# Banus/pano360

Measured on AMD Instinct MI355X. Metric: blended megapixels/sec (multiband), higher is better.
Workload: dtype f32; 1 GPU; cfg3: 32 synthetic 3840x2160 frames per image set, spherical warp + multiband blend L=5, native resolution (MAX_RESOLUTION uncapped); frames=32

## Files before the change

### pano360_amd/csrc/blend.hip

```cpp
#include <stdlib.h>

#include "geom.h"

__global__ __launch_bounds__(256) void ownership_kernel(
    const pano_patch *__restrict__ patches, int n, int H, int W,
    int16_t *__restrict__ owner, uint8_t *__restrict__ valid) {
    const int x = blockIdx.x * 64 + threadIdx.x, y = blockIdx.y * 4 + threadIdx.y;
    if (x >= W || y >= H) return;
    float best = 0.0f;
    int who = -1;
    bool any = false;
    for (int i = 0; i < n; ++i) {
        const pano_patch p = patches[i];
        const int px = x - p.x0, py = y - p.y0;
        if ((unsigned)px >= (unsigned)p.w || (unsigned)py >= (unsigned)p.h) continue;
        const float a = p.planes[3 * (size_t)p.vh * p.vpitch + (size_t)py * p.vpitch + px];
        if (a > best) {
            best = a;
            who = i;
        }
        any |= p.mask[(size_t)py * p.w + px] == 0;
    }
    owner[(size_t)y * W + x] = (int16_t)who;
    valid[(size_t)y * W + x] = any ? 1 : 0;
}

#define OWN_LIST 256

struct CamList {
    int list[OWN_LIST];
    int wave[4];
    int count;
};

__device__ __forceinline__ int build_camera_list(CamList &sh, const pano_camera *__restrict__ cams,
                                                 int n, int bx0, int bx1, int by0, int by1) {
    const int tid = threadIdx.y * 64 + threadIdx.x, lane = threadIdx.x, wave = threadIdx.y;
    if (tid == 0) sh.count = 0;
    __syncthreads();
    bool overflow = false;
    for (int base = 0; base < n; base += 256) {
        const int i = base + tid;
        bool hit = false;
        if (i < n) {
            const pano_camera *cam = cams + i;
            hit = cam->x0 < bx1 && cam->x0 + cam->w > bx0 && cam->y0 < by1 && cam->y0 + cam->h > by0;
        }
        const unsigned long long bal = __ballot(hit);
        if (lane == 0) sh.wave[wave] = __popcll(bal);
        __syncthreads();
        int off = sh.count;
        for (int w = 0; w < wave; ++w) off += sh.wave[w];
        const int total = sh.count + sh.wave[0] + sh.wave[1] + sh.wave[2] + sh.wave[3];
        off += __popcll(bal & ((1ull << lane) - 1ull));
        if (hit && off < OWN_LIST) sh.list[off] = i;
        __syncthreads();
        if (tid == 0) sh.count = total;
        if (total > OWN_LIST) overflow = true;
        __syncthreads();
    }
    return overflow ? -1 : sh.count;
}

struct AlphaBound {
    float lo, hi;
};

__device__ __forceinline__ void hat_range(double a, double b, int n, double &lo, double &hi) {
    const double mid = 0.5 * n, peak = fmin(fmax(mid, a), b);
    hi = 0.5 - fabs(peak - mid) / n;
    lo = fmin(0.5 - fabs(a - mid) / n, 0.5 - fabs(b - mid) / n);
}

__device__ __forceinline__ void iv_axpy(double k, double lo, double hi, double &alo, double &ahi) {
    alo += k >= 0.0 ? k * lo : k * hi;
    ahi += k >= 0.0 ? k * hi : k * lo;
}

__device__ __forceinline__ AlphaBound alpha_bound_of(const pano_camera *cam, const double (*v)[2]);

__device__ __forceinline__ AlphaBound alpha_bound(const pano_camera *cam, const double *r) {
    const double *K = cam->proj;
    double v[3][2];
#pragma unroll
    for (int row = 0; row < 3; ++row) {
        double lo = 0.0, hi = 0.0;
        iv_axpy(K[3 * row + 0], r[0], r[1], lo, hi);
        iv_axpy(K[3 * row + 1], r[2], r[3], lo, hi);
        iv_axpy(K[3 * row + 2], r[4], r[5], lo, hi);
        const double slack = 1e-9 * (fabs(lo) + fabs(hi)) + 1e-300;
        v[row][0] = lo - slack;
        v[row][1] = hi + slack;
    }
    return alpha_bound_of(cam, v);
}

__device__ __forceinline__ AlphaBound alpha_bound_ends(const pano_camera *cam, double sa, double ca,
                                                       double sb, double cb, double t_lo,
                                                       double t_hi) {
    const double *K = cam->proj;
    const double chord2 = (sb - sa) * (sb - sa) + (cb - ca) * (cb - ca);
    double v[3][2];
#pragma unroll
    for (int row = 0; row < 3; ++row) {
        const double a = K[3 * row + 0], b = K[3 * row + 2];
        const double ga = a * sa + b * ca, gb = a * sb + b * cb;
        const double e = (fabs(a) + fabs(b)) * chord2 * 0.1258;
        double lo = fmin(ga, gb) - e, hi = fmax(ga, gb) + e;
        iv_axpy(K[3 * row + 1], t_lo, t_hi, lo, hi);
        const double slack = 1e-9 * (fabs(lo) + fabs(hi) + fabs(ga) + fabs(gb)) + 1e-300;
        v[row][0] = lo - slack;
        v[row][1] = hi + slack;
    }
    return alpha_bound_of(cam, v);
}

__device__ __forceinline__ AlphaBound alpha_bound_of(const pano_camera *cam, const double (*v)[2]) {
    AlphaBound out;
    if (v[2][1] <= 0.0) {
        out.lo = 0.0f;
        out.hi = -1.0f;
        return out;
    }
    if (v[2][0] <= 1e-6 * (fabs(v[0][0]) + fabs(v[0][1]) + fabs(v[1][0]) + fabs(v[1][1]) + 1.0)) {
        out.lo = 0.0f;
        out.hi = 1.0f;
        return out;
    }
    const int sw = cam->sw, sh = cam->sh;
    double box[2][2];
#pragma unroll
    for (int a = 0; a < 2; ++a) {
        const double q0 = v[a][0] / v[2][0], q1 = v[a][0] / v[2][1];
        const double q2 = v[a][1] / v[2][0], q3 = v[a][1] / v[2][1];
        const double half = 0.5 * (a == 0 ? sw : sh);
        box[a][0] = fmin(fmin(q0, q1), fmin(q2, q3)) + half - 2.0;
        box[a][1] = fmax(fmax(q0, q1), fmax(q2, q3)) + half + 2.0;
    }
    if (box[0][1] < 0.0 || box[0][0] > sw - 1.0 || box[1][1] < 0.0 || box[1][0] > sh - 1.0) {
        out.lo = 0.0f;
        out.hi = -1.0f;
        return out;
    }
    const bool inside = box[0][0] >= 0.0 && box[0][1] <= sw - 1.0 && box[1][0] >= 0.0 &&
                        box[1][1] <= sh - 1.0;
    double xlo, xhi, ylo, yhi;
    hat_range(fmax(box[0][0], 0.0), fmin(box[0][1], sw - 1.0), sw, xlo, xhi);
    hat_range(fmax(box[1][0], 0.0), fmin(box[1][1], sh - 1.0), sh, ylo, yhi);
    out.hi = (float)(fmax(xhi, 0.0) * fmax(yhi, 0.0) * (1.0 + 1e-6)) + 1e-7f;
    out.lo = inside ? fmaxf((float)(fmax(xlo, 0.0) * fmax(ylo, 0.0) * (1.0 - 1e-6)) - 1e-7f, 0.0f)
                    : 0.0f;
    return out;
}
// ... 363 lines not shown
        owned_box_pixel(o, x, y, top || row[x - W] != o, bottom || row[x + W] != o,
                        x == xs0 || row[x - 1] != o, x == xs1 - 1 || row[x + 1] != o, W, boxes,
                        stride, marks);
    }
}

__device__ __forceinline__ uint8_t quant255(float v) { return (uint8_t)(int)(255.0f * v); }

#define IB PANO_INTERIOR_BLOCK

__global__ __launch_bounds__(256) void block_owner_kernel(const int16_t *__restrict__ owner,
                                                          int H, int W, int xs0, int xs1,
                                                          int H8, int W8, int blo, int bhi,
                                                          int16_t *__restrict__ bown) {
    const int bx = blo + blockIdx.x * 64 + threadIdx.x, by = blockIdx.y * 4 + threadIdx.y;
    if (bx >= bhi || by >= H8) return;
    const int x0 = bx * IB, y0 = by * IB;
    int o = -2;
    if (x0 >= xs0 && (x0 + IB < W ? x0 + IB : W) <= xs1) {
        o = owner[(size_t)y0 * W + x0];
        const bool whole = x0 + IB <= W && (W & 1) == 0;
        if (x0 + IB <= W && y0 + IB <= H) {
            static_assert(IB == 4, "one 8-byte load per block row");
            typedef uint64_t u64_any __attribute__((aligned(2)));
            const uint64_t o16 = (uint16_t)o;
            const uint64_t all = o16 | o16 << 16 | o16 << 32 | o16 << 48;
            uint64_t diff = 0;
#pragma unroll
            for (int dy = 0; dy < IB; ++dy)
                diff |= *(const u64_any *)(owner + (size_t)(y0 + dy) * W + x0) ^ all;
            if (diff) o = -2;
        } else
        for (int dy = 0; dy < IB && o != -2; ++dy) {
            const int y = y0 + dy;
            if (y >= H) break;
            if (whole) {
                const uint32_t *q = (const uint32_t *)(owner + (size_t)y * W + x0);
                const uint32_t both = ((uint32_t)(uint16_t)o << 16) | (uint16_t)o;
                uint32_t diff = 0;
#pragma unroll
                for (int k = 0; k < IB / 2; ++k) diff |= q[k] ^ both;
                if (diff) o = -2;
            } else {
                for (int dx = 0; dx < IB; ++dx) {
                    const int x = x0 + dx;
                    if (x >= W) break;
                    if (owner[(size_t)y * W + x] != o) {
                        o = -2;
                        break;
                    }
                }
            }
        }
    }
    bown[(size_t)by * W8 + bx] = (int16_t)o;
}

#define IT_W 64
#define IT_H 16
#define IT_REACH_MAX 20
__device__ __forceinline__ bool agree(int a, int b) { return a == b || a == -3 || b == -3; }

struct LevelReaches {
    int n;
    int reach[PANO_MAX_LEVELS];
};

__global__ __launch_bounds__(256) void interior_tile_kernel(const int16_t *__restrict__ bown,
                                                            int H8, int W8, int reach, int blo,
                                                            int bhi, int ilo, int ihi,
                                                            uint8_t *__restrict__ interior,
                                                            LevelReaches lv,
                                                            uint8_t *__restrict__ classes) {
    __shared__ int16_t s_own[(IT_H + 2 * IT_REACH_MAX) * (IT_W + 2 * IT_REACH_MAX)];
    __shared__ int16_t s_col[IT_H * (IT_W + 2 * IT_REACH_MAX)];
    __shared__ unsigned long long s_vmask[IT_W + 2 * IT_REACH_MAX];
    const int tid = threadIdx.x, lane = tid & 63, wave = tid >> 6;
    const int bx0 = ilo + blockIdx.x * IT_W, by0 = blockIdx.y * IT_H;
    const int tw = IT_W + 2 * reach, th = IT_H + 2 * reach;
    for (int ty = wave; ty < th; ty += 4) {
        const int y = by0 - reach + ty;
        const bool row_in = y >= 0 && y < H8;
        for (int tx = lane; tx < tw; tx += 64) {
            const int x = bx0 - reach + tx;
            s_own[ty * tw + tx] = (row_in && x >= 0 && x < W8)
                                      ? (x >= blo && x < bhi ? bown[(size_t)y * W8 + x] : (int16_t)-2)
                                      : (int16_t)-3;
        }
    }
    __syncthreads();
    for (int tx = tid; tx < tw; tx += 256) {
        unsigned long long m = 0;
        int prev = s_own[tx];
#pragma unroll 8
        for (int ty = 0; ty + 1 < th; ++ty) {
            const int cur = s_own[(ty + 1) * tw + tx];
            m |= (unsigned long long)agree(prev, cur) << ty;
            prev = cur;
        }
        s_vmask[tx] = m;
    }
    __syncthreads();
    int cls[IT_H / 4];
#pragma unroll
    for (int r = 0; r < IT_H / 4; ++r) cls[r] = 0;
    const int nlv = classes ? lv.n : 1;
    for (int q = 0; q < nlv; ++q) {
        const int rq = classes ? lv.reach[q] : reach, off = reach - rq;
        const unsigned long long full = (1ull << (2 * rq)) - 1ull;
        for (int ry = wave; ry < IT_H; ry += 4)
            for (int tx = lane; tx < tw; tx += 64) {
                const int o = s_own[(ry + reach) * tw + tx];
                const bool same = ((s_vmask[tx] >> (ry + off)) & full) == full;
                s_col[ry * tw + tx] = (int16_t)(o >= 0 && !same ? -2 : o);
            }
        __syncthreads();
#pragma unroll
        for (int r = 0; r < IT_H / 4; ++r) {
            const int ry = wave + 4 * r;
            const int16_t *row = s_col + ry * tw;
            const int a0 = row[lane], a1 = row[min(lane + 1, tw - 1)];
            const int b0 = row[min(lane + 64, tw - 1)], b1 = row[min(lane + 65, tw - 1)];
            const unsigned long long lo = __ballot(lane + 1 < tw && agree(a0, a1));
            const unsigned long long hi = __ballot(lane + 65 < tw && agree(b0, b1));
            const int sh = lane + off;
            const unsigned long long win = sh == 0 ? lo
                                           : sh < 64 ? (lo >> sh) | (hi << (64 - sh))
                                                     : hi >> (sh - 64);
            const int o = row[lane + reach];
            if (o >= 0 && (win & full) == full && cls[r] == q) cls[r] = q + 1;
        }
        __syncthreads();
    }
#pragma unroll
    for (int r = 0; r < IT_H / 4; ++r) {
        const int y = by0 + wave + 4 * r, x = bx0 + lane;
        if (y >= H8 || x >= ihi) continue;
        interior[(size_t)y * W8 + x] = cls[r] == nlv ? 1 : 0;
        if (classes) classes[(size_t)y * W8 + x] = (uint8_t)cls[r];
    }
}

struct InteriorArgs {
    const uint8_t *interior;
    int W8;
    const pano_camera *cams;
    const double *sin_t, *cos_t, *tan_p;
    const float *lut;
    const uint8_t *classes;
};

enum { LUT_LDS = 0, LUT_GLOBAL = 1 };

template <int LUT>
__device__ __forceinline__ void shade_interior(const pano_camera *cam, const float *__restrict__ table,
                                               const InteriorArgs &ia, int x, int y, int W,
                                               uint8_t *__restrict__ mosaic,
                                               float *__restrict__ mosaic_f32) {
    if (!cam->frame) return;
    const int sw = cam->sw, sh = cam->sh;
    float fx, fy;
    map_pixel(cam->proj, table_f64(ia.sin_t, x), table_f64(ia.cos_t, x), table_f64(ia.tan_p, y), sw, sh, fx, fy);
    Taps tp = tap_base(fx, fy);
    TapBytes tb;
    if (__ballot(!taps_interior(tp, sw, sh)) == 0ull) {
        tb = load_taps_interior(cam->frame, sw, tp);
    } else {
        tp.x1 = min(tp.x1, sw - 1);
        tp.y1 = min(tp.y1, sh - 1);
        tb = load_taps(cam->frame, sw, tp);
    }
    const size_t g = ((size_t)y * W + x) * 3;
#pragma unroll
    for (int c = 0; c < 3; ++c) {
        float v = lerp4(lut_at(table, tb.v[0][c]), lut_at(table, tb.v[1][c]),
                        lut_at(table, tb.v[2][c]), lut_at(table, tb.v[3][c]), tp);
        v = v < 0.0f ? 0.0f : (v > 1.0f ? 1.0f : v);
        if (mosaic_f32) mosaic_f32[g + c] = v;
        mosaic[g + c] = (uint8_t)(int)(255.0f * v);
    }
}

template <int LUT>
__device__ __forceinline__ void shade_interior_of(int own, const float *__restrict__ table, int stride,
                                                  const InteriorArgs &ia, int x, int y, int W,
                                                  uint8_t *__restrict__ mosaic,
                                                  float *__restrict__ mosaic_f32) {
    const int own_u = __builtin_amdgcn_readfirstlane(own);
    if (__ballot(own != own_u) == 0)
        shade_interior<LUT>(ia.cams + own_u, table + (size_t)own_u * stride, ia, x, y, W, mosaic, mosaic_f32);
    else
        shade_interior<LUT>(ia.cams + own, table + (size_t)own * stride, ia, x, y, W, mosaic, mosaic_f32);
}

#define COMPOSE_MASKS 4
template <int L, bool PERCAM, bool CLS>
__global__ __launch_bounds__(256) void multiband_compose_kernel(
    const pano_patch *__restrict__ patches, int n, int H, int W, int xs0, int xs1,
    const int16_t *__restrict__ owner, const uint8_t *__restrict__ valid,
    uint8_t *__restrict__ mosaic, float *__restrict__ mosaic_f32, InteriorArgs ia) {
    __shared__ float s_lut[256];
    if (ia.interior && !PERCAM) {
        s_lut[threadIdx.y * 64 + threadIdx.x] = ia.lut[threadIdx.y * 64 + threadIdx.x];
        __syncthreads();
    }
    const int x = xs0 + blockIdx.x * 64 + threadIdx.x, y = blockIdx.y * 4 + threadIdx.y;
    const bool inside = x < xs1 && y < H;
    const bool is_interior = inside && ia.interior && ia.interior[(size_t)(y / IB) * ia.W8 + x / IB];
    unsigned long long cand[COMPOSE_MASKS] = {};
    const bool masked = n <= 64 * COMPOSE_MASKS && __ballot(inside && !is_interior) != 0;
    if (masked) {
        const int wx0 = xs0 + blockIdx.x * 64, wx1 = min(wx0 + 64, xs1);
#pragma unroll
        for (int m = 0; m < COMPOSE_MASKS; ++m) {
            const int i = 64 * m + (int)threadIdx.x;
            bool hit = false;
            if (i < n) {
                const pano_patch *q = patches + i;
                const int ax = q->x0 + q->ax0, ay = q->y0 + q->ay0;
                hit = ax < wx1 && ax + q->aw > wx0 && ay <= y && y < ay + q->ah;
            }
            cand[m] = __ballot(hit);
        }
    }
    if (!inside) return;
    if (is_interior) {
        const int own = owner[(size_t)y * W + x];
        if (PERCAM)
            shade_interior_of<LUT_GLOBAL>(own, ia.lut, 256, ia, x, y, W, mosaic, mosaic_f32);
        else
            shade_interior_of<LUT_LDS>(own, s_lut, 0, ia, x, y, W, mosaic, mosaic_f32);
        return;
    }
    float layer[L][3], wsum[L];
#pragma unroll
    for (int k = 0; k < L; ++k) layer[k][0] = layer[k][1] = layer[k][2] = wsum[k] = 0.0f;
    const int j = CLS && L > 1 ? (int)ia.classes[(size_t)(y / IB) * ia.W8 + x / IB] : 0;
    const int own_px = CLS && j > 0 ? (int)owner[(size_t)y * W + x] : -1;
    float base[3] = {0.0f, 0.0f, 0.0f};

    int m = 0;
    unsigned long long bits = masked ? cand[0] : 0ull;
    for (int i = 0;; ++i) {
        if (masked) {
            while (bits == 0ull && ++m < COMPOSE_MASKS) bits = cand[m];
            if (bits == 0ull) break;
            i = 64 * m + __ffsll((long long)bits) - 1;
            bits &= bits - 1ull;
        } else if (i >= n) {
            break;
        }
        const pano_patch p = patches[i];
        const int ax = x - p.x0 - p.ax0, ay = y - p.y0 - p.ay0;
        if ((unsigned)ax >= (unsigned)p.aw || (unsigned)ay >= (unsigned)p.ah) continue;
        const size_t vplane = (size_t)p.vh * p.vpitch;
        const size_t vo = (size_t)(ay + p.ay0 - p.vy0) * p.vpitch + (ax + p.ax0 - p.vx0);
        const size_t aplane = (size_t)p.ah * p.apitch, ao = (size_t)ay * p.apitch + ax;
        float hi[3], ha = 0.0f;
        if (!CLS || j == 0) {
#pragma unroll
            for (int c = 0; c < 3; ++c) hi[c] = p.planes[c * vplane + vo];
        } else {
            const float *b = p.blurred + (size_t)(j - 1) * 4 * aplane + ao;
#pragma unroll
            for (int c = 0; c < 3; ++c) hi[c] = b[c * aplane];
            if (p.index == own_px) {
#pragma unroll
                for (int c = 0; c < 3; ++c) base[c] = p.planes[c * vplane + vo] - hi[c];
            }
        }
        if (L == 1) ha = owner[(size_t)y * W + x] == p.index ? 1.0f : 0.0f;
#pragma unroll
        for (int k = 0; k < L; ++k) {
            if (CLS && k < j) continue;
            float rgb[3], a;
            if (k < L - 1) {
                const float *b = p.blurred + (size_t)k * 4 * aplane + ao;
                a = b[3 * aplane];
#pragma unroll
                for (int c = 0; c < 3; ++c) {
                    const float g = b[c * aplane];
                    rgb[c] = hi[c] - g;
                    hi[c] = g;
                }
                ha = a;
            } else {
                a = ha;
#pragma unroll
                for (int c = 0; c < 3; ++c) rgb[c] = hi[c];
            }
#pragma unroll
            for (int c = 0; c < 3; ++c) layer[k][c] = layer[k][c] + rgb[c] * a;
            wsum[k] = wsum[k] + a;
        }
    }
    const bool ok = valid[(size_t)y * W + x] != 0;
    float out[3] = {CLS && ok ? base[0] : 0.0f, CLS && ok ? base[1] : 0.0f, CLS && ok ? base[2] : 0.0f};
#pragma unroll
    for (int k = 0; k < L; ++k) {
        if (CLS && k < j) continue;
        const float ws = wsum[k] == 0.0f ? 1.0f : wsum[k];
#pragma unroll
        for (int c = 0; c < 3; ++c)
            out[c] = out[c] + __fdiv_rn(ok ? layer[k][c] : 0.0f, ws);
    }
    const size_t g = ((size_t)y * W + x) * 3;
#pragma unroll
    for (int c = 0; c < 3; ++c) {
        float v = out[c];
        v = v < 0.0f ? 0.0f : (v > 1.0f ? 1.0f : v);
        if (mosaic_f32) mosaic_f32[g + c] = v;
        mosaic[g + c] = quant255(v);
    }
}

__global__ __launch_bounds__(256) void linear_blend_kernel(
    const pano_patch *__restrict__ patches, int n, int H, int W,
    uint8_t *__restrict__ mosaic) {
    const int x = blockIdx.x * 64 + threadIdx.x, y = blockIdx.y * 4 + threadIdx.y;
    if (x >= W || y >= H) return;
    float acc[3] = {0.0f, 0.0f, 0.0f}, wsum = 0.0f;
    for (int i = 0; i < n; ++i) {
        const pano_patch p = patches[i];
        const int px = x - p.x0, py = y - p.y0;
        if ((unsigned)px >= (unsigned)p.w || (unsigned)py >= (unsigned)p.h) continue;
        const size_t plane = (size_t)p.vh * p.vpitch, o = (size_t)py * p.vpitch + px;
        const bool m = p.mask[(size_t)py * p.w + px] != 0;
        const float a = p.planes[3 * plane + o];
#pragma unroll
        for (int c = 0; c < 3; ++c) {
            const float t = m ? 0.0f : p.planes[c * plane + o];
            acc[c] = acc[c] + t * a;
        }
        wsum = wsum + a;
    }
    const float ws = wsum == 0.0f ? 1.0f : wsum;
    const size_t g = ((size_t)y * W + x) * 3;
#pragma unroll
    for (int c = 0; c < 3; ++c) mosaic[g + c] = quant255(__fdiv_rn(acc[c], ws));
}

__global__ __launch_bounds__(256) void no_blend_kernel(
    const pano_patch *__restrict__ patches, int n, int H, int W,
    uint8_t *__restrict__ mosaic) {
    const int x = blockIdx.x * 64 + threadIdx.x, y = blockIdx.y * 4 + threadIdx.y;
    if (x >= W || y >= H) return;
    uint8_t out[3] = {0, 0, 0};
    for (int i = 0; i < n; ++i) {
        const pano_patch p = patches[i];
        const int px = x - p.x0, py = y - p.y0;
        if ((unsigned)px >= (unsigned)p.w || (unsigned)py >= (unsigned)p.h) continue;
        if (p.mask[(size_t)py * p.w + px]) continue;
        const size_t plane = (size_t)p.vh * p.vpitch, o = (size_t)py * p.vpitch + px;
#pragma unroll
        for (int c = 0; c < 3; ++c) out[c] = quant255(p.planes[c * plane + o]);
    }
    const size_t g = ((size_t)y * W + x) * 3;
    mosaic[g] = out[0];
    mosaic[g + 1] = out[1];
    mosaic[g + 2] = out[2];
}

static int check_table(const void *table, int n, int H, int W, const char *who) {
    PANO_REQUIRE(table, "%s: null table", who);
    PANO_REQUIRE(n >= 0 && n <= 32767, "%s: %d patches (int16 owner map holds 32767)", who, n);
    PANO_REQUIRE(H > 0 && W > 0, "%s: bad mosaic shape %dx%d", who, H, W);
    return PANO_OK;
}

#define MOSAIC_GRID dim3 block(64, 4), grid(ceil_div(W, 64), ceil_div(H, 4))

extern "C" int pano_ownership(pano_ctx *ctx, const pano_patch *patches, int n, int H, int W,
                              int16_t *owner, uint8_t *valid) {
    PANO_ENTER(ctx, "pano_ownership");
    if (int rc = check_table(patches, n, H, W, "pano_ownership")) return rc;
    PANO_REQUIRE(owner && valid, "pano_ownership: null output");
    MOSAIC_GRID;
    PANO_TIMED(PK_OWNERSHIP, (hipStream_t)stream,
               hipLaunchKernelGGL(ownership_kernel, grid, block, 0, (hipStream_t)stream,
                                  patches, n, H, W, owner, valid));
    PANO_LAUNCH_CHECK("ownership_kernel");
    return PANO_OK;
}

extern "C" int pano_ownership_cameras(pano_ctx *ctx, const pano_camera *cams, int n, int H, int W,
                                      int xs0, int xs1, const double *sin_t, const double *cos_t,
                                      const double *tan_p, int16_t *owner, uint8_t *valid) {
    PANO_ENTER(ctx, "pano_ownership_cameras");
    if (int rc = check_table(cams, n, H, W, "pano_ownership_cameras")) return rc;
    PANO_REQUIRE(sin_t && cos_t && tan_p && owner && valid, "pano_ownership_cameras: null pointer");
    PANO_REQUIRE(xs0 >= 0 && xs1 <= W && xs0 <= xs1, "pano_ownership_cameras: bad strip [%d, %d)", xs0, xs1);
    if (xs0 == xs1) return PANO_OK;
    const int prune = ctx->opt[PANO_OPT_OWN_PRUNE];
    dim3 block(64, 4), grid(ceil_div(xs1 - xs0, 64), ceil_div(H, (prune & 2) ? OWN_TILE_ROWS : OW_TH_TALL));
    PANO_TIMED(PK_OWNERSHIP_CAMS, (hipStream_t)stream,
               hipLaunchKernelGGL((prune & 2) ? ownership_cameras_l1_kernel : ownership_cameras_kernel,
                                  grid, block, (prune & 2) ? 0 : own_shared_bytes(n),
                                  (hipStream_t)stream, cams, n, H, W, xs0, xs1, sin_t, cos_t,
                                  tan_p, owner, valid, prune & 1, (int32_t *)nullptr, 0,
                                  (uint8_t *)nullptr));
    PANO_LAUNCH_CHECK("ownership_cameras_kernel");
    return PANO_OK;
}

extern "C" int pano_blend_cameras(pano_ctx *ctx, const pano_camera *cams, int n, int H, int W,
                                  int xs0, int xs1, int linear, const double *sin_t,
                                  const double *cos_t, const double *tan_p, const float *lut,
                                  int lut_stride, uint8_t *mosaic, uint8_t *valid) {
    PANO_ENTER(ctx, "pano_blend_cameras");
    if (int rc = check_table(cams, n, H, W, "pano_blend_cameras")) return rc;
    PANO_REQUIRE(sin_t && cos_t && tan_p && lut && mosaic, "pano_blend_cameras: null pointer");
    PANO_REQUIRE(lut_stride == 0 || lut_stride == 256,
                 "pano_blend_cameras: lut_stride %d (0 = shared table, 256 = per camera)", lut_stride);
    PANO_REQUIRE(xs0 >= 0 && xs1 <= W && xs0 <= xs1, "pano_blend_cameras: bad strip [%d, %d)", xs0, xs1);
    if (xs0 == xs1) return PANO_OK;
    dim3 block(64, 4), grid(ceil_div(xs1 - xs0, 64), ceil_div(H, 4));
    hipStream_t s = (hipStream_t)stream;
#define BLEND(LIN, PC)                                                                        \
    PANO_TIMED(PK_BLEND_CAMERAS, s,                                                           \
               hipLaunchKernelGGL((blend_cameras_kernel<LIN, PC>), grid, block, 0, s, cams, n, \
                                  H, W, xs0, xs1, sin_t, cos_t, tan_p, lut, mosaic, valid))
    if (linear && lut_stride) BLEND(true, true);
    else if (linear) BLEND(true, false);
    else if (lut_stride) BLEND(false, true);
    else BLEND(false, false);
#undef BLEND
    PANO_LAUNCH_CHECK("blend_cameras_kernel");
    return PANO_OK;
}

#define SPAN_WORDS 1024
__global__ __launch_bounds__(256) void owned_spans_kernel(const uint8_t *__restrict__ marks,
                                                          int W, int xs0, int xs1, int min_gap,
                                                          int max_spans, int stride,
                                                          int32_t *__restrict__ regions) {
    __shared__ unsigned long long s_bits[SPAN_WORDS];
    const int lane = threadIdx.x & 63, wave = threadIdx.x >> 6;
    const uint8_t *row = marks + (size_t)blockIdx.x * W;
    int32_t *out = regions + (size_t)blockIdx.x * stride + 5;
    int cnt = 0, last = 0;
    const int32_t *box = regions + (size_t)blockIdx.x * stride;
    xs0 = max(xs0, box[2]);
    xs1 = min(xs1, box[3] + 1);
    for (int chunk0 = xs0; chunk0 < xs1; chunk0 += 64 * SPAN_WORDS) {
        const int words = min(SPAN_WORDS, (xs1 - chunk0 + 63) >> 6);
        for (int w = wave; w < words; w += 4) {
            const int x = chunk0 + 64 * w + lane;
            const unsigned long long bal = __ballot(x < xs1 && row[x] != 0);
            if (lane == 0) s_bits[w] = bal;
        }
        __syncthreads();
        if (wave == 0) {
            for (int w = 0; w < words; ++w) {
                const int base = chunk0 + 64 * w;
                unsigned long long bal = s_bits[w];
                while (bal) {
                    const int s = __ffsll((long long)bal) - 1;
                    const unsigned long long rest = ~(bal >> s);
                    const int len = rest ? __ffsll((long long)rest) - 1 : 64 - s;
                    const int xa = base + s, xb = xa + len - 1;
                    if (cnt && (xa - last - 1 < min_gap || cnt == max_spans)) {
                        if (lane == 0) out[2 * (cnt - 1) + 1] = xb;
                    } else {
                        if (lane == 0) {
                            out[2 * cnt] = xa;
// ... 25 lines not shown
    const size_t words = mark_bytes / 16, step = (size_t)gridDim.x * 256;
    uint4 *m16 = (uint4 *)marks;
    for (size_t k = i; k < words; k += step) m16[k] = make_uint4(0u, 0u, 0u, 0u);
    if (i < mark_bytes - words * 16) marks[words * 16 + i] = 0;
}

static int launch_init_regions(hipStream_t s, int32_t *regions, int n, int stride, uint8_t *marks,
                               int W) {
    size_t bytes = (size_t)n * W;
    if ((uintptr_t)marks & 15) {
        PANO_HIP(hipMemsetAsync(marks, 0, bytes, s));
        bytes = 0;
    }
    const size_t want = bytes / 16 / 256 + 1;
    const int blocks = (int)(want < 2048 ? (want > (size_t)ceil_div(n, 256) ? want : ceil_div(n, 256))
                                         : 2048);
    hipLaunchKernelGGL(init_regions_kernel, dim3(blocks), dim3(256), 0, s, regions, n, stride, marks,
                       bytes);
    PANO_LAUNCH_CHECK("init_regions_kernel");
    return PANO_OK;
}

extern "C" int pano_owned_regions(pano_ctx *ctx, const int16_t *owner, int H, int W, int xs0,
                                  int xs1, int n, int min_gap, int max_spans, uint8_t *marks,
                                  int32_t *regions) {
    PANO_ENTER(ctx, "pano_owned_regions");
    PANO_REQUIRE(owner && marks && regions, "pano_owned_regions: null pointer");
    PANO_REQUIRE(H > 0 && W > 0 && n >= 0 && n <= 32767 && max_spans >= 1 && min_gap >= 0,
                 "pano_owned_regions: bad argument");
    PANO_REQUIRE(xs0 >= 0 && xs1 <= W && xs0 <= xs1, "pano_owned_regions: bad strip [%d, %d)", xs0, xs1);
    if (n == 0) return PANO_OK;
    hipStream_t s = (hipStream_t)stream;
    const int stride = 5 + 2 * max_spans;
    if (int rc = launch_init_regions(s, regions, n, stride, marks, W)) return rc;
    if (xs0 == xs1) return PANO_OK;
    dim3 block(64, 4), grid(ceil_div(xs1 - xs0, 512), ceil_div(H, 4));
    PANO_TIMED(PK_OWNED_BOXES, s,
               hipLaunchKernelGGL(owned_boxes_kernel, grid, block, 0, s, owner, H, W, xs0, xs1,
                                  regions, stride, marks));
    PANO_LAUNCH_CHECK("owned_boxes_kernel");
    PANO_TIMED(PK_OWNED_SPANS, s,
               hipLaunchKernelGGL(owned_spans_kernel, dim3(n), dim3(256), 0, s, marks, W, xs0, xs1,
                                  min_gap, max_spans, stride, regions));
    PANO_LAUNCH_CHECK("owned_spans_kernel");
    return PANO_OK;
}

extern "C" int pano_ownership_regions(pano_ctx *ctx, const pano_camera *cams, int n, int H, int W,
                                      int xs0, int xs1, const double *sin_t, const double *cos_t,
                                      const double *tan_p, int16_t *owner, uint8_t *valid,
                                      int min_gap, int max_spans, uint8_t *marks,
                                      int32_t *regions) {
    PANO_ENTER(ctx, "pano_ownership_regions");
    if (int rc = check_table(cams, n, H, W, "pano_ownership_regions")) return rc;
    PANO_REQUIRE(sin_t && cos_t && tan_p && owner && valid && marks && regions,
                 "pano_ownership_regions: null pointer");
    PANO_REQUIRE(xs0 >= 0 && xs1 <= W && xs0 <= xs1, "pano_ownership_regions: bad strip [%d, %d)", xs0, xs1);
    PANO_REQUIRE(max_spans >= 1 && min_gap >= 0, "pano_ownership_regions: bad argument");
    if (n == 0) return PANO_OK;
    hipStream_t s = (hipStream_t)stream;
    const int stride = 5 + 2 * max_spans;
    if (int rc = launch_init_regions(s, regions, n, stride, marks, W)) return rc;
    if (xs0 == xs1) return PANO_OK;
    const int prune = ctx->opt[PANO_OPT_OWN_PRUNE];
    dim3 block(64, 4), grid(ceil_div(xs1 - xs0, 64), ceil_div(H, (prune & 2) ? OWN_TILE_ROWS : OW_TH_TALL));
    PANO_TIMED(PK_OWNERSHIP_CAMS, s,
               hipLaunchKernelGGL((prune & 2) ? ownership_cameras_l1_kernel : ownership_cameras_kernel,
                                  grid, block, (prune & 2) ? 0 : own_shared_bytes(n), s, cams, n, H, W, xs0,
                                  xs1, sin_t, cos_t, tan_p, owner, valid, prune & 1, regions, stride,
                                  marks));
    PANO_LAUNCH_CHECK("ownership_cameras_kernel");
    PANO_TIMED(PK_OWNED_SPANS, s,
               hipLaunchKernelGGL(owned_spans_kernel, dim3(n), dim3(256), 0, s, marks, W, xs0, xs1,
                                  min_gap, max_spans, stride, regions));
    PANO_LAUNCH_CHECK("owned_spans_kernel");
    return PANO_OK;
}

static int interior_map_launch(pano_ctx *ctx, const int16_t *owner, int H, int W, int xs0, int xs1,
                               const int *radii, int n_radii, int16_t *block_owner,
                               uint8_t *interior, uint8_t *classes, const char *who) {
    void *const stream = (void *)ctx->stream;
    PANO_REQUIRE(owner && block_owner && interior && radii, "%s: null pointer", who);
    PANO_REQUIRE(H > 0 && W > 0 && n_radii >= 1 && n_radii < PANO_MAX_LEVELS, "%s: bad argument", who);
    PANO_REQUIRE(xs0 >= 0 && xs1 <= W && xs0 <= xs1, "%s: bad strip [%d, %d)", who, xs0, xs1);
    LevelReaches lv = {};
    lv.n = n_radii;
    for (int k = 0; k < n_radii; ++k) {
        PANO_REQUIRE(radii[k] >= 0 && (k == 0 || radii[k] >= radii[k - 1]),
                     "%s: radii must ascend (level %d: %d)", who, k, radii[k]);
        lv.reach[k] = ceil_div(radii[k] + IB - 1, IB);
    }
    const int radius = radii[n_radii - 1];
    const int H8 = ceil_div(H, IB), W8 = ceil_div(W, IB), reach = lv.reach[n_radii - 1];
    if (xs0 == xs1) return PANO_OK;
    const int ilo = xs0 / IB, ihi = ceil_div(xs1, IB);
    const int blo = ilo - reach > 0 ? ilo - reach : 0, bhi = ihi + reach < W8 ? ihi + reach : W8;
    dim3 block(64, 4), grid(ceil_div(bhi - blo, 64), ceil_div(H8, 4));
    hipStream_t s = (hipStream_t)stream;
    PANO_TIMED(PK_INTERIOR, s,
               hipLaunchKernelGGL(block_owner_kernel, grid, block, 0, s, owner, H, W, xs0, xs1,
                                  H8, W8, blo, bhi, block_owner));
    PANO_LAUNCH_CHECK("block_owner_kernel");
    PANO_REQUIRE(reach <= IT_REACH_MAX, "%s: radius %d reaches %d blocks (at most %d)", who, radius,
                 reach, IT_REACH_MAX);
    hipLaunchKernelGGL(interior_tile_kernel, dim3(ceil_div(ihi - ilo, IT_W), ceil_div(H8, IT_H)),
                       dim3(256), 0, s, block_owner, H8, W8, reach, blo, bhi, ilo, ihi, interior, lv,
                       classes);
    PANO_LAUNCH_CHECK("interior_tile_kernel");
    return PANO_OK;
}

extern "C" int pano_interior_map(pano_ctx *ctx, const int16_t *owner, int H, int W, int xs0,
                                 int xs1, int radius, int16_t *block_owner, uint8_t *interior) {
    PANO_ENTER(ctx, "pano_interior_map");
    return interior_map_launch(ctx, owner, H, W, xs0, xs1, &radius, 1, block_owner, interior, nullptr,
                               "pano_interior_map");
}

extern "C" int pano_interior_classes(pano_ctx *ctx, const int16_t *owner, int H, int W, int xs0,
                                     int xs1, const int *radii, int n_radii, int16_t *block_owner,
                                     uint8_t *interior, uint8_t *classes) {
    PANO_ENTER(ctx, "pano_interior_classes");
    PANO_REQUIRE(classes, "pano_interior_classes: null pointer");
    return interior_map_launch(ctx, owner, H, W, xs0, xs1, radii, n_radii, block_owner, interior,
                               classes, "pano_interior_classes");
}

extern "C" int pano_multiband_compose(pano_ctx *ctx, const pano_patch *patches, int n, int H,
                                      int W, int xs0, int xs1, int n_levels, const int16_t *owner,
                                      const uint8_t *valid, const uint8_t *interior,
                                      const uint8_t *classes, const pano_camera *cams,
                                      const double *sin_t,
                                      const double *cos_t, const double *tan_p, const float *lut,
                                      int lut_stride, uint8_t *mosaic, float *mosaic_f32) {
    PANO_ENTER(ctx, "pano_multiband_compose");
    if (int rc = check_table(patches, n, H, W, "pano_multiband_compose")) return rc;
    PANO_REQUIRE(H > 0 && W > 0, "pano_multiband_compose: bad mosaic shape %dx%d", H, W);
    PANO_REQUIRE(owner && mosaic && valid, "pano_multiband_compose: null pointer");
    PANO_REQUIRE(n_levels >= 1 && n_levels <= PANO_MAX_LEVELS,
                 "pano_multiband_compose: n_levels %d outside [1, %d]", n_levels, PANO_MAX_LEVELS);
    PANO_REQUIRE(xs0 >= 0 && xs1 <= W && xs0 <= xs1,
                 "pano_multiband_compose: bad strip [%d, %d)", xs0, xs1);
    PANO_REQUIRE(!interior || (cams && sin_t && cos_t && tan_p && lut),
                 "pano_multiband_compose: the interior map needs cameras, tables and LUT");
    PANO_REQUIRE(lut_stride == 0 || lut_stride == 256,
                 "pano_multiband_compose: lut_stride %d (0 = shared table, 256 = per camera)",
                 lut_stride);
    if (xs0 == xs1) return PANO_OK;
    PANO_REQUIRE(!classes || interior, "pano_multiband_compose: level classes without the interior map");
    InteriorArgs ia = {interior, ceil_div(W, IB), cams, sin_t, cos_t, tan_p, lut,
                       ctx->opt[PANO_OPT_LEVEL_CLASSES] ? classes : nullptr};
    const bool percam = interior && lut_stride != 0;
    dim3 block(64, 4), grid(ceil_div(xs1 - xs0, 64), ceil_div(H, 4));
    hipStream_t s = (hipStream_t)stream;
#define COMPOSE_AS(L, PC, CL)                                                            \
    PANO_TIMED(PK_COMPOSE, s,                                                           \
               hipLaunchKernelGGL((multiband_compose_kernel<L, PC, CL>), grid, block, 0, s, \
                                  patches, n, H, W, xs0, xs1, owner, valid, mosaic,     \
                                  mosaic_f32, ia))
#define COMPOSE(L)                                                                      \
    case L:                                                                             \
        if (ia.classes && L > 1) {                                                      \
            if (percam) COMPOSE_AS(L, true, true); else COMPOSE_AS(L, false, true);     \
        } else {                                                                        \
            if (percam) COMPOSE_AS(L, true, false); else COMPOSE_AS(L, false, false);   \
        }                                                                               \
        break;
    switch (n_levels) {
        COMPOSE(1) COMPOSE(2) COMPOSE(3) COMPOSE(4) COMPOSE(5) COMPOSE(6) COMPOSE(7) COMPOSE(8)
    }
#undef COMPOSE_AS
#undef COMPOSE
    PANO_LAUNCH_CHECK("multiband_compose_kernel");
    return PANO_OK;
}

extern "C" int pano_linear_blend(pano_ctx *ctx, const pano_patch *patches, int n, int H, int W,
                                 uint8_t *mosaic) {
    PANO_ENTER(ctx, "pano_linear_blend");
    if (int rc = check_table(patches, n, H, W, "pano_linear_blend")) return rc;
    PANO_REQUIRE(mosaic, "pano_linear_blend: null output");
    MOSAIC_GRID;
    PANO_TIMED(PK_LINEAR, (hipStream_t)stream,
               hipLaunchKernelGGL(linear_blend_kernel, grid, block, 0, (hipStream_t)stream,
                                  patches, n, H, W, mosaic));
    PANO_LAUNCH_CHECK("linear_blend_kernel");
    return PANO_OK;
}

extern "C" int pano_no_blend(pano_ctx *ctx, const pano_patch *patches, int n, int H, int W,
                             uint8_t *mosaic) {
    PANO_ENTER(ctx, "pano_no_blend");
    if (int rc = check_table(patches, n, H, W, "pano_no_blend")) return rc;
    PANO_REQUIRE(mosaic, "pano_no_blend: null output");
    MOSAIC_GRID;
    PANO_TIMED(PK_NOBLEND, (hipStream_t)stream,
               hipLaunchKernelGGL(no_blend_kernel, grid, block, 0, (hipStream_t)stream,
                                  patches, n, H, W, mosaic));
    PANO_LAUNCH_CHECK("no_blend_kernel");
    return PANO_OK;
}
```

Measured before the change: 215,200 MP/s.

## Process two rows per thread in multiband compose and hoist per-pixel loads

Each compose thread now handles two vertically adjacent pixels, sharing the sin/cos table reads, the interior-map lookup, the candidate-patch ballot and the camera projection matrix across both rows. When the wave has a single owner, the camera parameters are pinned to scalar registers. Owner and valid loads are issued up front, and the launch bounds gain a per-level occupancy hint. The aim is to cut redundant loads and per-thread setup in exchange for more registers per thread and half as many blocks.

```diff
diff --git a/pano360_amd/csrc/blend.hip b/pano360_amd/csrc/blend.hip
--- a/pano360_amd/csrc/blend.hip
+++ b/pano360_amd/csrc/blend.hip
@@ -1,4 +1,5 @@
 #include <stdlib.h>
+#include <type_traits>
 
 #include "geom.h"
 
@@ -668,50 +669,92 @@
 
 enum { LUT_LDS = 0, LUT_GLOBAL = 1 };
 
-template <int LUT>
-__device__ __forceinline__ void shade_interior(const pano_camera *cam, const float *__restrict__ table,
-                                               const InteriorArgs &ia, int x, int y, int W,
+#define COMPOSE_ROWS 2
+static_assert(IB % COMPOSE_ROWS == 0, "a thread's rows lie in one interior cell");
+
+typedef const __attribute__((address_space(4))) pano_camera *uniform_camera;
+template <int LUT, int NR, typename Cam>
+__device__ __forceinline__ void shade_interior(Cam cam, const float *__restrict__ table,
+                                               int x, int y0, int H, int W, double s, double c,
+                                               const double *t,
                                                uint8_t *__restrict__ mosaic,
                                                float *__restrict__ mosaic_f32) {
-    if (!cam->frame) return;
-    const int sw = cam->sw, sh = cam->sh;
-    float fx, fy;
-    map_pixel(cam->proj, table_f64(ia.sin_t, x), table_f64(ia.cos_t, x), table_f64(ia.tan_p, y), sw, sh, fx, fy);
-    Taps tp = tap_base(fx, fy);
-    TapBytes tb;
-    if (__ballot(!taps_interior(tp, sw, sh)) == 0ull) {
-        tb = load_taps_interior(cam->frame, sw, tp);
+    const uint8_t *frame = cam->frame;
+    int sw = cam->sw, sh = cam->sh;
+    double K[9];
+#pragma unroll
+    for (int k = 0; k < 9; ++k) K[k] = cam->proj[k];
+    if constexpr (std::is_same<Cam, uniform_camera>::value)
+        asm volatile("" : "+s"(frame), "+s"(sw), "+s"(sh), "+s"(K[0]), "+s"(K[1]), "+s"(K[2]), "+s"(K[3]),
+                          "+s"(K[4]), "+s"(K[5]), "+s"(K[6]), "+s"(K[7]), "+s"(K[8]));
+    else
+        asm volatile("" : "+v"(frame), "+v"(sw), "+v"(sh), "+v"(K[0]), "+v"(K[1]), "+v"(K[2]), "+v"(K[3]),
+                          "+v"(K[4]), "+v"(K[5]), "+v"(K[6]), "+v"(K[7]), "+v"(K[8]));
+    if (!frame) return;
+    Taps tp[NR];
+    TapBytes tb[NR];
+    bool inner = true;
+#pragma unroll
+    for (int r = 0; r < NR; ++r) {
+        float fx, fy;
+        map_pixel(K, s, c, t[r], sw, sh, fx, fy);
+        tp[r] = tap_base(fx, fy);
+        inner &= taps_interior(tp[r], sw, sh);
+    }
+    if (__ballot(!inner) == 0ull) {
+#pragma unroll
+        for (int r = 0; r < NR; ++r) tb[r] = load_taps_interior(frame, sw, tp[r]);
     } else {
-        tp.x1 = min(tp.x1, sw - 1);
-        tp.y1 = min(tp.y1, sh - 1);
-        tb = load_taps(cam->frame, sw, tp);
-    }
-    const size_t g = ((size_t)y * W + x) * 3;
-#pragma unroll
-    for (int c = 0; c < 3; ++c) {
-        float v = lerp4(lut_at(table, tb.v[0][c]), lut_at(table, tb.v[1][c]),
-                        lut_at(table, tb.v[2][c]), lut_at(table, tb.v[3][c]), tp);
-        v = v < 0.0f ? 0.0f : (v > 1.0f ? 1.0f : v);
-        if (mosaic_f32) mosaic_f32[g + c] = v;
-        mosaic[g + c] = (uint8_t)(int)(255.0f * v);
+#pragma unroll
+        for (int r = 0; r < NR; ++r) {
+            tp[r].x1 = min(tp[r].x1, sw - 1);
+            tp[r].y1 = min(tp[r].y1, sh - 1);
+            tb[r] = load_taps(frame, sw, tp[r]);
+        }
+    }
+#pragma unroll
+    for (int r = 0; r < NR; ++r) {
+        if (y0 + r >= H) break;
+        const size_t g = ((size_t)(y0 + r) * W + x) * 3;
+#pragma unroll
+        for (int ch = 0; ch < 3; ++ch) {
+            float v = lerp4(lut_at(table, tb[r].v[0][ch]), lut_at(table, tb[r].v[1][ch]),
+                            lut_at(table, tb[r].v[2][ch]), lut_at(table, tb[r].v[3][ch]), tp[r]);
+            v = v < 0.0f ? 0.0f : (v > 1.0f ? 1.0f : v);
+            if (mosaic_f32) mosaic_f32[g + ch] = v;
+            mosaic[g + ch] = (uint8_t)(int)(255.0f * v);
+        }
     }
 }
 
 template <int LUT>
 __device__ __forceinline__ void shade_interior_of(int own, const float *__restrict__ table, int stride,
-                                                  const InteriorArgs &ia, int x, int y, int W,
+                                                  const InteriorArgs &ia, int x, int y0, int H, int W,
+                                                  double s, double c, const double *t,
                                                   uint8_t *__restrict__ mosaic,
                                                   float *__restrict__ mosaic_f32) {
     const int own_u = __builtin_amdgcn_readfirstlane(own);
-    if (__ballot(own != own_u) == 0)
-        shade_interior<LUT>(ia.cams + own_u, table + (size_t)own_u * stride, ia, x, y, W, mosaic, mosaic_f32);
-    else
-        shade_interior<LUT>(ia.cams + own, table + (size_t)own * stride, ia, x, y, W, mosaic, mosaic_f32);
+    if (__ballot(own != own_u) == 0) {
+        shade_interior<LUT, COMPOSE_ROWS>((uniform_camera)(ia.cams + own_u), table + (size_t)own_u * stride,
+                                          x, y0, H, W, s, c, t, mosaic, mosaic_f32);
+    } else {
+#pragma unroll 1
+        for (int r = 0; r < COMPOSE_ROWS; ++r) {
+            double tr = t[0];
+#pragma unroll
+            for (int q = 1; q < COMPOSE_ROWS; ++q) tr = r == q ? t[q] : tr;
+            shade_interior<LUT, 1>(ia.cams + own, table + (size_t)own * stride, x, y0 + r, H, W, s, c,
+                                   &tr, mosaic, mosaic_f32);
+        }
+    }
 }
 
 #define COMPOSE_MASKS 4
+constexpr int compose_waves(int L, bool CLS) {
+    return L <= 5 ? 8 : L == 6 ? (CLS ? 7 : 8) : L == 7 ? 6 : 5;
+}
 template <int L, bool PERCAM, bool CLS>
-__global__ __launch_bounds__(256) void multiband_compose_kernel(
+__global__ __launch_bounds__(256, compose_waves(L, CLS)) void multiband_compose_kernel(
     const pano_patch *__restrict__ patches, int n, int H, int W, int xs0, int xs1,
     const int16_t *__restrict__ owner, const uint8_t *__restrict__ valid,
     uint8_t *__restrict__ mosaic, float *__restrict__ mosaic_f32, InteriorArgs ia) {
@@ -720,9 +763,27 @@
         s_lut[threadIdx.y * 64 + threadIdx.x] = ia.lut[threadIdx.y * 64 + threadIdx.x];
         __syncthreads();
     }
-    const int x = xs0 + blockIdx.x * 64 + threadIdx.x, y = blockIdx.y * 4 + threadIdx.y;
-    const bool inside = x < xs1 && y < H;
-    const bool is_interior = inside && ia.interior && ia.interior[(size_t)(y / IB) * ia.W8 + x / IB];
+    int x = xs0 + blockIdx.x * 64 + threadIdx.x;
+    const int y0 = (blockIdx.y * 4 + threadIdx.y) * COMPOSE_ROWS;
+    const int xc = min(x, xs1 - 1);
+    int yc[COMPOSE_ROWS];
+#pragma unroll
+    for (int r = 0; r < COMPOSE_ROWS; ++r) yc[r] = min(y0 + r, H - 1);
+    int own = owner[(size_t)yc[0] * W + xc];
+    unsigned ok_rows = 0;
+#pragma unroll
+    for (int r = 0; r < COMPOSE_ROWS; ++r) ok_rows |= (valid[(size_t)yc[r] * W + xc] != 0 ? 1u : 0u) << r;
+    unsigned flag = 0;
+    double s = 0.0, c = 0.0, t[COMPOSE_ROWS] = {};
+    if (ia.interior) {
+        flag = ia.interior[(size_t)(yc[0] / IB) * ia.W8 + xc / IB];
+        s = table_f64(ia.sin_t, xc);
+        c = table_f64(ia.cos_t, xc);
+#pragma unroll
+        for (int r = 0; r < COMPOSE_ROWS; ++r) t[r] = table_f64(ia.tan_p, yc[r]);
+    }
+    const bool inside = x < xs1 && y0 < H;
+    const bool is_interior = inside && flag;
     unsigned long long cand[COMPOSE_MASKS] = {};
     const bool masked = n <= 64 * COMPOSE_MASKS && __ballot(inside && !is_interior) != 0;
     if (masked) {
@@ -734,99 +795,104 @@
             if (i < n) {
                 const pano_patch *q = patches + i;
                 const int ax = q->x0 + q->ax0, ay = q->y0 + q->ay0;
-                hit = ax < wx1 && ax + q->aw > wx0 && ay <= y && y < ay + q->ah;
+                hit = ax < wx1 && ax + q->aw > wx0 && ay < y0 + COMPOSE_ROWS && y0 < ay + q->ah;
             }
             cand[m] = __ballot(hit);
         }
     }
     if (!inside) return;
     if (is_interior) {
-        const int own = owner[(size_t)y * W + x];
         if (PERCAM)
-            shade_interior_of<LUT_GLOBAL>(own, ia.lut, 256, ia, x, y, W, mosaic, mosaic_f32);
+            shade_interior_of<LUT_GLOBAL>(own, ia.lut, 256, ia, x, y0, H, W, s, c, t, mosaic, mosaic_f32);
         else
-            shade_interior_of<LUT_LDS>(own, s_lut, 0, ia, x, y, W, mosaic, mosaic_f32);
+            shade_interior_of<LUT_LDS>(own, s_lut, 0, ia, x, y0, H, W, s, c, t, mosaic, mosaic_f32);
         return;
     }
-    float layer[L][3], wsum[L];
-#pragma unroll
-    for (int k = 0; k < L; ++k) layer[k][0] = layer[k][1] = layer[k][2] = wsum[k] = 0.0f;
-    const int j = CLS && L > 1 ? (int)ia.classes[(size_t)(y / IB) * ia.W8 + x / IB] : 0;
-    const int own_px = CLS && j > 0 ? (int)owner[(size_t)y * W + x] : -1;
-    float base[3] = {0.0f, 0.0f, 0.0f};
-
-    int m = 0;
-    unsigned long long bits = masked ? cand[0] : 0ull;
-    for (int i = 0;; ++i) {
-        if (masked) {
-            while (bits == 0ull && ++m < COMPOSE_MASKS) bits = cand[m];
-            if (bits == 0ull) break;
-            i = 64 * m + __ffsll((long long)bits) - 1;
-            bits &= bits - 1ull;
-        } else if (i >= n) {
-            break;
-        }
-        const pano_patch p = patches[i];
-        const int ax = x - p.x0 - p.ax0, ay = y - p.y0 - p.ay0;
-        if ((unsigned)ax >= (unsigned)p.aw || (unsigned)ay >= (unsigned)p.ah) continue;
-        const size_t vplane = (size_t)p.vh * p.vpitch;
-        const size_t vo = (size_t)(ay + p.ay0 - p.vy0) * p.vpitch + (ax + p.ax0 - p.vx0);
-        const size_t aplane = (size_t)p.ah * p.apitch, ao = (size_t)ay * p.apitch + ax;
-        float hi[3], ha = 0.0f;
-        if (!CLS || j == 0) {
-#pragma unroll
-            for (int c = 0; c < 3; ++c) hi[c] = p.planes[c * vplane + vo];
-        } else {
-            const float *b = p.blurred + (size_t)(j - 1) * 4 * aplane + ao;
-#pragma unroll
-            for (int c = 0; c < 3; ++c) hi[c] = b[c * aplane];
-            if (p.index == own_px) {
-#pragma unroll
-                for (int c = 0; c < 3; ++c) base[c] = p.planes[c * vplane + vo] - hi[c];
-            }
-        }
-        if (L == 1) ha = owner[(size_t)y * W + x] == p.index ? 1.0f : 0.0f;
+    const int j = CLS && L > 1 ? (int)ia.classes[(size_t)(y0 / IB) * ia.W8 + x / IB] : 0;
+#pragma unroll 1
+    for (int r = 0; r < COMPOSE_ROWS; ++r) {
+        const int y = y0 + r;
+        if (y >= H) break;
+        asm volatile("" : "+v"(x));
+        float layer[L][3], wsum[L];
+#pragma unroll
+        for (int k = 0; k < L; ++k) layer[k][0] = layer[k][1] = layer[k][2] = wsum[k] = 0.0f;
+        const int own_px = CLS && j > 0 ? (int)owner[(size_t)y * W + x] : -1;
+        float base[3] = {0.0f, 0.0f, 0.0f};
+
+        int m = 0;
+        unsigned long long bits = masked ? cand[0] : 0ull;
+        for (int i = 0;; ++i) {
+            if (masked) {
+                while (bits == 0ull && ++m < COMPOSE_MASKS) bits = cand[m];
+                if (bits == 0ull) break;
+                i = 64 * m + __ffsll((long long)bits) - 1;
+                bits &= bits - 1ull;
+            } else if (i >= n) {
+                break;
+            }
+            const pano_patch p = patches[i];
+            const int ax = x - p.x0 - p.ax0, ay = y - p.y0 - p.ay0;
+            if ((unsigned)ax >= (unsigned)p.aw || (unsigned)ay >= (unsigned)p.ah) continue;
+            const size_t vplane = (size_t)p.vh * p.vpitch;
+            const size_t vo = (size_t)(ay + p.ay0 - p.vy0) * p.vpitch + (ax + p.ax0 - p.vx0);
+            const size_t aplane = (size_t)p.ah * p.apitch, ao = (size_t)ay * p.apitch + ax;
+            float hi[3], ha = 0.0f;
+            if (!CLS || j == 0) {
+#pragma unroll
+                for (int c = 0; c < 3; ++c) hi[c] = p.planes[c * vplane + vo];
+            } else {
+                const float *b = p.blurred + (size_t)(j - 1) * 4 * aplane + ao;
+#pragma unroll
+                for (int c = 0; c < 3; ++c) hi[c] = b[c * aplane];
+                if (p.index == own_px) {
+#pragma unroll
+                    for (int c = 0; c < 3; ++c) base[c] = p.planes[c * vplane + vo] - hi[c];
+                }
+            }
+            if (L == 1) ha = owner[(size_t)y * W + x] == p.index ? 1.0f : 0.0f;
+#pragma unroll
+            for (int k = 0; k < L; ++k) {
+                if (CLS && k < j) continue;
+                float rgb[3], a;
+                if (k < L - 1) {
+                    const float *b = p.blurred + (size_t)k * 4 * aplane + ao;
+                    a = b[3 * aplane];
+#pragma unroll
+                    for (int c = 0; c < 3; ++c) {
+                        const float g = b[c * aplane];
+                        rgb[c] = hi[c] - g;
+                        hi[c] = g;
+                    }
+                    ha = a;
+                } else {
+                    a = ha;
+#pragma unroll
+                    for (int c = 0; c < 3; ++c) rgb[c] = hi[c];
+                }
+#pragma unroll
+                for (int c = 0; c < 3; ++c) layer[k][c] = layer[k][c] + rgb[c] * a;
+                wsum[k] = wsum[k] + a;
+            }
+        }
+        const bool ok = (ok_rows >> r & 1u) != 0;
+        float out[3] = {CLS && ok ? base[0] : 0.0f, CLS && ok ? base[1] : 0.0f, CLS && ok ? base[2] : 0.0f};
 #pragma unroll
         for (int k = 0; k < L; ++k) {
             if (CLS && k < j) continue;
-            float rgb[3], a;
-            if (k < L - 1) {
-                const float *b = p.blurred + (size_t)k * 4 * aplane + ao;
-                a = b[3 * aplane];
-#pragma unroll
-                for (int c = 0; c < 3; ++c) {
-                    const float g = b[c * aplane];
-                    rgb[c] = hi[c] - g;
-                    hi[c] = g;
-                }
-                ha = a;
-            } else {
-                a = ha;
-#pragma unroll
-                for (int c = 0; c < 3; ++c) rgb[c] = hi[c];
-            }
-#pragma unroll
-            for (int c = 0; c < 3; ++c) layer[k][c] = layer[k][c] + rgb[c] * a;
-            wsum[k] = wsum[k] + a;
-        }
-    }
-    const bool ok = valid[(size_t)y * W + x] != 0;
-    float out[3] = {CLS && ok ? base[0] : 0.0f, CLS && ok ? base[1] : 0.0f, CLS && ok ? base[2] : 0.0f};
-#pragma unroll
-    for (int k = 0; k < L; ++k) {
-        if (CLS && k < j) continue;
-        const float ws = wsum[k] == 0.0f ? 1.0f : wsum[k];
-#pragma unroll
-        for (int c = 0; c < 3; ++c)
-            out[c] = out[c] + __fdiv_rn(ok ? layer[k][c] : 0.0f, ws);
-    }
-    const size_t g = ((size_t)y * W + x) * 3;
-#pragma unroll
-    for (int c = 0; c < 3; ++c) {
-        float v = out[c];
-        v = v < 0.0f ? 0.0f : (v > 1.0f ? 1.0f : v);
-        if (mosaic_f32) mosaic_f32[g + c] = v;
-        mosaic[g + c] = quant255(v);
+            const float ws = wsum[k] == 0.0f ? 1.0f : wsum[k];
+#pragma unroll
+            for (int c = 0; c < 3; ++c)
+                out[c] = out[c] + __fdiv_rn(ok ? layer[k][c] : 0.0f, ws);
+        }
+        const size_t g = ((size_t)y * W + x) * 3;
+#pragma unroll
+        for (int c = 0; c < 3; ++c) {
+            float v = out[c];
+            v = v < 0.0f ? 0.0f : (v > 1.0f ? 1.0f : v);
+            if (mosaic_f32) mosaic_f32[g + c] = v;
+            mosaic[g + c] = quant255(v);
+        }
     }
 }
 
@@ -1158,7 +1224,7 @@
     InteriorArgs ia = {interior, ceil_div(W, IB), cams, sin_t, cos_t, tan_p, lut,
                        ctx->opt[PANO_OPT_LEVEL_CLASSES] ? classes : nullptr};
     const bool percam = interior && lut_stride != 0;
-    dim3 block(64, 4), grid(ceil_div(xs1 - xs0, 64), ceil_div(H, 4));
+    dim3 block(64, 4), grid(ceil_div(xs1 - xs0, 64), ceil_div(H, 4 * COMPOSE_ROWS));
     hipStream_t s = (hipStream_t)stream;
 #define COMPOSE_AS(L, PC, CL)                                                            \
     PANO_TIMED(PK_COMPOSE, s,                                                           \
```

Result: faster. 225,900 MP/s (median of 6 runs) (+5.0%).
